# youthHan/HVRNet

Measured on AMD Instinct MI355X. Metric: VID frames/sec, R101 Faster-RCNN+HVR, 1000x600, 300 props, T=15, higher is better.
Workload: dtype bf16; 1 GPU; configs[2]: faster_rcnn_r101_hrnmp_c5 inference, clip mode; frames_per_window=15, proposals_per_frame=300, input=3x600x1000 padded to 608x1008, parallelism=dp1 independent clips, no collectives, windows_in_flight=12, clips_per_graph=3, key_frame_detections=300

## Files before the change

### hvrnet_amd/backbone.py

```python
import torch
import torch.nn as nn

from . import native
from .registry import BACKBONES, SHARED_HEADS

ARCH_SETTINGS = {50: (3, 4, 6, 3), 101: (3, 4, 23, 3), 152: (3, 8, 36, 3)}
STEM_KP = 192


def as_nhwc(x, dtype):
    v = x.permute(0, 2, 3, 1)
    if v.is_contiguous():
        return v if x.dtype == dtype else native.cast(v, dtype)
    return native.nchw_to_nhwc(x.contiguous(), dtype)


def as_logical(y):
    return y.permute(0, 3, 1, 2)


def fold_conv_bn(conv, bn, dtype):
    if bn is not None and conv.bias is None and dtype == torch.bfloat16 and conv.weight.is_cuda \
            and conv.weight.dtype == torch.float32 and conv.weight.is_contiguous() and not bn.training:
        from . import train_ops as TO
# ... 219 lines not shown
            if isinstance(m, nn.Conv2d):
                nn.init.kaiming_normal_(m.weight, mode='fan_out', nonlinearity='relu')
            elif isinstance(m, nn.BatchNorm2d):
                nn.init.constant_(m.weight, 1)
                nn.init.constant_(m.bias, 0)
        if self.zero_init_residual:
            for m in self.modules():
                if isinstance(m, Bottleneck):
                    nn.init.constant_(m.bn3.weight, 0)
        set_compute_dtype(self, self.compute_dtype)

    def _pack(self, dtype):
        w, b = fold_conv_bn(self.conv1, self.bn1, torch.float32)
        wp = torch.zeros((64, STEM_KP), dtype=torch.float32, device=w.device)
        wp[:, :147] = w.reshape(64, 147)
        wf = torch.zeros((64, 7, 8, 4), dtype=torch.float32, device=w.device)
        wf[:, :, :7, :3] = w
        if dtype == native.SPLIT:
            fused, fused_bias = native.stem_split_weights(wf.view(64, 7, 32)), native.stem_split_bias(b)
        else:
            fused, fused_bias = wf.view(64, 7, 32).to(dtype if dtype in (torch.bfloat16, torch.float16) else torch.bfloat16).contiguous(), b
        return dict(stem=(native.as_operand(wp, dtype), b), fused=fused, fused_bias=fused_bias)

    def out_shape_nhwc(self, B, H, W):
        if len(self.out_indices) != 1:
            return None
        last = self.out_indices[0]
        h, w = (H + 6 - 7) // 2 + 1, (W + 6 - 7) // 2 + 1
        h, w = (h + 2 - 3) // 2 + 1, (w + 2 - 3) // 2 + 1
        for i in range(last + 1):
            h, w = (h - 1) // self.strides[i] + 1, (w - 1) // self.strides[i] + 1
        return (B, h, w, 64 * 2 ** last * 4)

    def forward(self, x, out=None):
        if not x.is_cuda:
            raise NotImplementedError('ResNet runs on the GPU only (no CPU fallback)')
        p = self.packed(x.device)
        dt = self.compute_dtype
        if dt in (torch.bfloat16, torch.float16, native.SPLIT) and self.fused_stem:
            y = native.stem_fused(x.contiguous().float(), p['fused'], p['fused_bias'])
        else:
            cols, OH, OW = native.im2col_stem(x.contiguous().float(), dt, STEM_KP)
            if dt == native.SPLIT:
                y = native.gemm(cols, p['stem'][0], p['stem'][1], relu=True, out_f32=True).view(x.shape[0], OH, OW, 64)
                y = native.cast(native.maxpool3x3s2_nhwc(y), dt)
            else:
                y = native.gemm(cols, p['stem'][0], p['stem'][1], relu=True).view(x.shape[0], OH, OW, 64)
                y = native.maxpool3x3s2_nhwc(y)
        outs = []
        if out is not None:
            assert len(self.out_indices) == 1, 'out= needs a single returned map'
        for i, name in enumerate(self.res_layers):
            blocks = list(getattr(self, name))
            h1 = None
            for j, blk in enumerate(blocks):
                last = out is not None and i == self.out_indices[0] and j == len(blocks) - 1
                if j + 1 < len(blocks):
                    y, h1 = blk.forward_nhwc(y, h1=h1, nxt=blocks[j + 1])
                else:
                    y = blk.forward_nhwc(y, out=out if last else None, h1=h1)
            if i in self.out_indices:
                outs.append(as_logical(y))
            if out is not None and i == self.out_indices[0]:
                break
        return tuple(outs)

    def forward_train_nhwc(self, x):
        p = self.packed(x.device)
        dt = self.compute_dtype
        with torch.no_grad():
            if dt in (torch.bfloat16, torch.float16, native.SPLIT) and self.fused_stem:
                y = native.stem_fused(x.contiguous().float(), p['fused'], p['fused_bias'])
            else:
                cols, OH, OW = native.im2col_stem(x.contiguous().float(), dt, STEM_KP)
                y = native.gemm(cols, p['stem'][0], p['stem'][1], relu=True).view(x.shape[0], OH, OW, 64)
                y = native.maxpool3x3s2_nhwc(y)
            for i, name in enumerate(self.res_layers):
                if i + 1 <= self.frozen_stages:
                    for blk in getattr(self, name):
                        y = blk.forward_nhwc(y)
        for i, name in enumerate(self.res_layers):
            if i + 1 > self.frozen_stages:
                for blk in getattr(self, name):
                    y = blk.forward_train_nhwc(y)
        return y

    def train(self, mode=True):
# ... 67 lines not shown
```

### hvrnet_amd/csrc/capi.hip

```cpp
#include "../../include/hvr_hip.h"

#include <cmath>
#include <cstdarg>
#include <cstdio>
#include <cstdlib>
#include <cstring>
#include <string>

#include "common.h"
#include "gemm_params.h"
#include "relation_bt.h"

namespace hvr {
hipError_t run_transpose_pad(const void*, void*, int, int, long, long, int, hipStream_t);
hipError_t run_zero_fill(void*, size_t, hipStream_t);
hipError_t run_pack_conv_weights_multi(const void*, int, long, int, hipStream_t);
hipError_t run_transpose_multi(const void*, int, int, hipStream_t);
hipError_t run_im2col_t(const void*, void*, int, int, int, int, int, int, int, int, int, int, long, hipStream_t);
hipError_t run_relu_bwd_t(const void*, const void*, void*, void*, int, int, long, hipStream_t);
hipError_t run_splitk_reduce(const float*, float*, int, int, long, int, hipStream_t);
hipError_t run_unpack_conv_wgrads_multi(const void*, int, long, int, hipStream_t);
hipError_t run_splitk_reduce_bf16(const float*, void*, int, int, long, int, hipStream_t);
hipError_t run_splitk_reduce_f16(const float*, void*, int, int, long, int, hipStream_t);
hipError_t run_splitk_reduce_half_batched(const float*, void*, int, int, long, int, int, int, long, long, hipStream_t);
// ... 25 lines not shown
size_t tta_merge_proposals_workspace_bytes(int A, int T, int mx);
hipError_t run_tta_merge_proposals(const float*, const int*, int, int, int, const float*, const float*, const int*, float, int, float*, int*, void*,
                                   hipStream_t);
hipError_t run_tta_map_rois(const float*, int, int, int, const float*, const float*, const int*, float*, hipStream_t);
hipError_t run_tta_merge_dets(const float*, const float*, int, int, int, const float*, const float*, const int*, float*, float*, hipStream_t);
hipError_t run_mining_argreduce(const float*, int, int, long, const long long*, const long long*, long long*, hipStream_t);
hipError_t run_relation_dscore(const void*, const void*, const void*, const void*, void*, int, long, int, long, long, float, int, hipStream_t);
hipError_t run_im2col_stem(const float*, void*, int, int, int, int, int, int, int, hipStream_t);
hipError_t run_maxpool3x3s2(const void*, void*, int, int, int, int, int, int, int, hipStream_t);
hipError_t run_cast(const void*, void*, long, int, int, float, hipStream_t);
hipError_t run_permute(const void*, void*, int, int, int, int, int, int, hipStream_t);
hipError_t run_det_decode(const float*, int, int, int, int, const float*, int, const float*, const float*, float, float,
                          float, float, float*, float*, hipStream_t);
hipError_t run_roi_align_fwd(const void*, const float*, void*, int, int, int, int, int, int, int, float, int, int, int,
                             hipStream_t);
hipError_t run_roi_align_bwd(const float*, const float*, float*, int, int, int, int, int, int, float, int, int, hipStream_t);
size_t nms_workspace_bytes(int P, int n);
hipError_t run_nms_batched(const float*, int, int, float, int, int, int, long long*, int*, void*, hipStream_t, int band = 0,
                           int* band_done = nullptr);
hipError_t run_rpn_select(const void*, const void*, long, long, float*, const RpnParams&, int, hipStream_t);
hipError_t run_rpn_select_wide(const void*, const void*, long, long, float*, const RpnParams&, void*, hipStream_t);
size_t rpn_wide_workspace_bytes(int T, long n_anchor);
int rpn_wide_max_frames(int set);
int* rpn_wide_done_flags(void* wws, int T);
hipError_t run_rpn_gather(const float*, const long long*, const int*, int, int, int, int, int, float*, int*, hipStream_t);
hipError_t run_multiclass_nms(const float*, const float*, int, int, float, float, int, float*, long long*, int*, void*,
                              hipStream_t);
size_t multiclass_nms_workspace_bytes(int R, int ncls);
hipError_t run_soft_nms(const float*, int, float, int, float, float, float*, long long*, int*, hipStream_t);
hipError_t run_multiclass_soft_nms(const float*, const float*, int, int, int, float, float, int, float, float, int, float*, long long*, int*,
                                   void*, hipStream_t);
size_t multiclass_soft_nms_workspace_bytes(int P, int R, int ncls);
hipError_t run_stem_fused(const float*, const void*, const float*, void*, int, int, int, int, hipStream_t);
}

using namespace hvr;

static thread_local std::string g_err;

static int fail(int code, const char* fmt, ...) {
  char buf[512];
  va_list ap;
  va_start(ap, fmt);
  vsnprintf(buf, sizeof buf, fmt, ap);
  va_end(ap);
  g_err = buf;
  return code;
}
static int check_launch(hipError_t e, const char* what) {
  if (e == hipSuccess) return HVR_OK;
  if (e == hipErrorInvalidValue) return fail(HVR_EUNSUPPORTED, "%s: shape outside the implemented envelope", what);
  return fail(HVR_ELAUNCH, "%s: %s", what, hipGetErrorString(e));
}
static inline size_t align256(size_t b) { return (b + 255) & ~(size_t)255; }
static inline int elem_size(int dtype) { return (dtype == HVR_BF16 || dtype == HVR_F16) ? 2 : 4; }
static inline int kstep_elems(int dtype) { return (dtype == HVR_F32 || dtype == HVR_F16S) ? 32 : 64; }
static inline bool valid_dtype(int dtype) { return dtype >= HVR_F32 && dtype <= HVR_F16S; }
static inline bool aligned128(const void* p) { return (reinterpret_cast<uintptr_t>(p) & 127) == 0; }
static inline bool aligned16(const void* p) { return (reinterpret_cast<uintptr_t>(p) & 15) == 0; }

extern "C" {

int hvr_abi_version(void) { return 6; }
const char* hvr_last_error(void) { return g_err.c_str(); }

static int fill_linear(GemmParams& p, const void* A, const void* B, void* C, int M, int N, int K, long lda, long ldb,
// ... 366 lines not shown
    return fail(HVR_EUNSUPPORTED, "no fused tail + next conv kernel for C1=%d C2=%d Cout=%d Cn=%d", d->tail.C1, d->tail.C2, d->tail.Cout, d->Cn);
  return check_launch(run_expand(p, (hipStream_t)stream), "hvr_bottleneck_tail_next");
}

int hvr_conv2d_path(const hvr_conv_desc* d) {
  GemmParams p;
  int path = 0;
  const int rc = conv_params(d, p, path);
  if (rc) return rc;
  if (path == 0 && (d->tile_hint == 0 || d->tile_hint == kBigHint)) {
    p.tile_hint = 0;
    if (bigtile_supported(p, d->tile_hint == kBigHint)) return 3;
  }
  return path;
}

int hvr_im2col_stem(const float* img, void* cols, int B, int H, int W, int KP, int dtype, void* stream) {
  if (!img || !cols || B <= 0) return fail(HVR_EINVAL, "bad stem arguments");
  if (dtype == HVR_F16S && (KP % 32 || !aligned128(cols))) return fail(HVR_EINVAL, "split-half patch rows: KP %% 32 == 0, 128-byte aligned");
  if (KP < 147 || KP % kstep_elems(dtype)) return fail(HVR_EINVAL, "KP=%d must be >= 147 and a K-step multiple", KP);
  const int OH = (H + 6 - 7) / 2 + 1, OW = (W + 6 - 7) / 2 + 1;
  return check_launch(run_im2col_stem(img, cols, B, H, W, OH, OW, KP, dtype, (hipStream_t)stream), "hvr_im2col_stem");
}

int hvr_stem_fused_dtype(const float* img, const void* wpk, const float* bias, void* out, int B, int H, int W, int dtype, void* stream) {
  if (!img || !wpk || !bias || !out || B <= 0 || H < 7 || W < 7) return fail(HVR_EINVAL, "bad fused-stem arguments");
  if (dtype != HVR_BF16 && dtype != HVR_F16 && dtype != HVR_F16S) return fail(HVR_EUNSUPPORTED, "the fused stem computes on bf16, half or split-half operands");
  if (!aligned16(wpk) || !aligned16(out) || !aligned16(bias)) return fail(HVR_EINVAL, "fused stem operands must be 16-byte aligned");
  if (dtype == HVR_F16S && !aligned128(out)) return fail(HVR_EINVAL, "split-half stem output must be 128-byte aligned");
  return check_launch(run_stem_fused(img, wpk, bias, out, B, H, W, dtype, (hipStream_t)stream), "hvr_stem_fused");
}
int hvr_stem_fused(const float* img, const void* wpk, const float* bias, void* out, int B, int H, int W, void* stream) {
  return hvr_stem_fused_dtype(img, wpk, bias, out, B, H, W, HVR_BF16, stream);
}

int hvr_maxpool3x3s2_nhwc(const void* x, void* y, int B, int H, int W, int C, int dtype, void* stream) {
  if (!x || !y || C % 4) return fail(HVR_EINVAL, "bad maxpool arguments (C %% 4 == 0 required)");
  if (dtype == HVR_F16S) return fail(HVR_EUNSUPPORTED, "max pooling runs on f32 / bf16 / half maps");
  const int OH = (H + 2 - 3) / 2 + 1, OW = (W + 2 - 3) / 2 + 1;
  return check_launch(run_maxpool3x3s2(x, y, B, H, W, C, OH, OW, dtype, (hipStream_t)stream), "hvr_maxpool3x3s2_nhwc");
}

static int env_tile(const char* name) {
  const char* v = std::getenv(name);
  return v ? std::atoi(v) : 0;
}
static inline long rel_ldp(int Mk) { return ((long)Mk + 127) / 128 * 128; }

static int apply_slice_blocks() { return 4; }
static int apply_slices(int Mq, int Mk, int D) {
  const long tiles = (long)((Mq + 127) / 128) * ((D + 127) / 128);
  const int nblk = (int)(rel_ldp(Mk) / 128);
  if (tiles >= 96 || nblk < 8 || D % 8) return 1;
  const int per = apply_slice_blocks();
  return (nblk + per - 1) / per;
}

static int relation_apply_pass(const void* P, const void* Vt, float* mstat, float* lstat, float* partial, void* O, int64_t ldo,
                               int Mq, int Mk, int D, long ldp, int nt, int dtype, int staging, hipStream_t s) {
  const bool two_byte = dtype == HVR_BF16 || dtype == HVR_F16;
  constexpr int tile_apply = 0, gm_apply = 1;
#ifdef HVR_DEBUG_KNOBS
  static const int dbg_ld0 = env_tile("HVR_DBG_LD0");
#endif
  GemmParams p;
  int rc;
// ... 778 lines not shown
```

### hvrnet_amd/csrc/check_regs.py

```python
import re
import sys


def main(*paths):
    text = ''.join(open(p).read() for p in paths)
    blocks = re.split(r'remark: (?:\S+ )?Function Name: ', text)[1:]
    bad, seen = [], 0
    for b in blocks:
        name = b.split()[0]
        if name.startswith(('_ZN3hvr17expand_res_kernel', '_ZN3hvr19expand_split_kernel')):
            seen += 1
            spill = int(re.search(r'VGPRs Spill: (\d+)', b).group(1))
            scratch = int(re.search(r'ScratchSize \[bytes/lane\]: (\d+)', b).group(1))
            if spill or scratch:
                bad.append('%s: %d VGPRs spilled, %d bytes of scratch' % (name, spill, scratch))
            continue
        if name.startswith(('_ZN3hvr19mc_nms_', '_ZN3hvr15nms_', '_ZN3hvr16nms_', '_ZN3hvr17rpn_', '_ZN3hvr25relation_scores_bt', '_ZN3hvr14pc_tile_kernel', '_ZN3hvr15big_tile_kernel')) \
                or re.match(r'_ZN3hvr\d+(?:tta|soft_nms)_', name):
            seen += 1
            spill = int(re.search(r'VGPRs Spill: (\d+)', b).group(1))
            scratch = int(re.search(r'ScratchSize \[bytes/lane\]: (\d+)', b).group(1))
            allow = 32 if re.match(r'_ZN3hvr14pc_tile_kernelI(?:t|NS_5f16_tE)Li4ELi0E', name) else (256 if re.match(r'_ZN3hvr14pc_tile_kernelI(?:t|NS_5f16_tE)Li2ELi2E', name) else 0)
            if scratch > allow or (spill and not allow):
                bad.append('%s: %d VGPRs spilled, %d bytes of scratch' % (name, spill, scratch))
            continue
        m = re.match(r'_ZN3hvr11tile_kernelI(?:t|f|NS_5f16_tE|NS_6f16s_tE)Li(\d+)ELi(\d+)ELi(\d+)ELi(\d+)ELi(\d+)ELb([01])ELb([01])ELi(\d+)E', name)
        if not m:
            continue
        wm, wn, fm, fn, epi, glds, respre, ns = [int(x) for x in m.groups()]
        spill = int(re.search(r'VGPRs Spill: (\d+)', b).group(1))
        bn = wn * fn * 16
        split_pipe = 'f16s_t' in name and ns > 2 and not (wm == 3 and fn == 8)
        untracked = epi == 2 or (ns > 2 and respre == 1 and bn != 256) or split_pipe
        if untracked:
            seen += 1
            if spill:
                bad.append('%s: %d VGPRs spilled' % (name, spill))
    if not seen:
        sys.exit('check_regs: no kernel recognised in the remarks (format change?)')
    if bad:
        sys.exit('check_regs: these kernels must not spill:\n  ' + '\n  '.join(bad))
    print('check_regs: %d kernels checked (untracked loads / serial sweeps / big accumulator tiles), none spills' % seen)

# ... 4 lines not shown
```

### hvrnet_amd/csrc/stem.hip

```cpp
#include "common.h"

namespace hvr {

#ifndef HVR_ST_PH
#define HVR_ST_PH 3
#endif
#ifndef HVR_ST_PW
#define HVR_ST_PW 16
#endif
constexpr int ST_PH = HVR_ST_PH, ST_PW = HVR_ST_PW;
constexpr int ST_CH = 2 * ST_PH + 1, ST_CW = 2 * ST_PW + 1;
constexpr int ST_NCONV = ST_CH * ST_CW;
constexpr int ST_FRAGS = (ST_NCONV + 15) / 16;
constexpr int ST_IR = 2 * (ST_CH - 1) + 7, ST_IC = 2 * (ST_CW - 1) + 7;
constexpr int ST_PCOLS = 72;
constexpr int ST_CROW = 68;
constexpr int ST_PATCH_BYTES = (ST_IR + 3) * ST_PCOLS * 4 * 2;
constexpr int ST_CONV_BYTES = ST_FRAGS * 16 * ST_CROW * 2;

template <typename T>
__global__ __launch_bounds__(256) void stem_fused_kernel(const float* __restrict__ img, const uint4* __restrict__ wpk,
                                                         const float* __restrict__ bias, T* __restrict__ out, int H,
                                                         int W, int CH, int CW, int PH, int PW) {
  extern __shared__ __attribute__((aligned(16))) char smem[];
  T* patch = reinterpret_cast<T*>(smem);
  T* cbuf = reinterpret_cast<T*>(smem + ST_PATCH_BYTES);
  const int tid = threadIdx.x, lane = tid & 63, wave = tid >> 6;
  const int px0 = blockIdx.x * ST_PW, py0 = blockIdx.y * ST_PH, b = blockIdx.z;
  const int cy0 = 2 * py0 - 1, cx0 = 2 * px0 - 1;
  const int iy0 = 2 * cy0 - 3, ix0 = 2 * cx0 - 3;

  uint4 wf[4][7];
#pragma unroll
// ... 169 lines not shown

  for (int i = tid; i < ST_PH * ST_PW * 4; i += 256) {
    const int ch = i & 3, q = i >> 2, qy = q / ST_PW, qx = q - qy * ST_PW;
    const int py = py0 + qy, px = px0 + qx;
    if (py >= PH || px >= PW) continue;
    float best[8];
#pragma unroll
    for (int e = 0; e < 8; ++e) best[e] = -INFINITY;
#pragma unroll
    for (int dy = 0; dy < 3; ++dy) {
      const int gy = 2 * py - 1 + dy;
      if ((unsigned)gy >= (unsigned)CH) continue;
#pragma unroll
      for (int dx = 0; dx < 3; ++dx) {
        const int gx = 2 * px - 1 + dx;
        if ((unsigned)gx >= (unsigned)CW) continue;
        const float* src = cbuf + ((gy - cy0) * ST_CW + (gx - cx0)) * ST_CROWF + ch * 8;
        const float4 a = *reinterpret_cast<const float4*>(src), c = *reinterpret_cast<const float4*>(src + 4);
        best[0] = fmaxf(best[0], a.x); best[1] = fmaxf(best[1], a.y); best[2] = fmaxf(best[2], a.z); best[3] = fmaxf(best[3], a.w);
        best[4] = fmaxf(best[4], c.x); best[5] = fmaxf(best[5], c.y); best[6] = fmaxf(best[6], c.z); best[7] = fmaxf(best[7], c.w);
      }
    }
    uint4 h, l;
    split2(best[0], best[1], h.x, l.x); split2(best[2], best[3], h.y, l.y);
    split2(best[4], best[5], h.z, l.z); split2(best[6], best[7], h.w, l.w);
    char* dst = out + (((long)b * PH + py) * PW + px) * 256 + half * 128 + ch * 16;
    *reinterpret_cast<uint4*>(dst) = h;
    *reinterpret_cast<uint4*>(dst + kSplitPlane) = l;
  }
  __syncthreads();
  }
}

hipError_t run_stem_fused(const float* img, const void* wpk, const float* bias, void* out, int B, int H, int W, int dtype, hipStream_t s) {
  const int CH = (H + 6 - 7) / 2 + 1, CW = (W + 6 - 7) / 2 + 1;
  const int PH = (CH + 2 - 3) / 2 + 1, PW = (CW + 2 - 3) / 2 + 1;
  constexpr int lds = ST_PATCH_BYTES + ST_CONV_BYTES;
  static std::atomic<unsigned> attr_dev{0};
  per_device_once(attr_dev, [&] {
    (void)hipFuncSetAttribute(reinterpret_cast<const void*>(stem_fused_kernel<bf16_t>), hipFuncAttributeMaxDynamicSharedMemorySize, lds);
    (void)hipFuncSetAttribute(reinterpret_cast<const void*>(stem_fused_kernel<f16_t>), hipFuncAttributeMaxDynamicSharedMemorySize, lds);
  });
  dim3 grid((PW + ST_PW - 1) / ST_PW, (PH + ST_PH - 1) / ST_PH, B);
  if (dtype == DT_F16S) {
    static std::atomic<unsigned> sattr_dev{0};
    per_device_once(sattr_dev, [&] {
      (void)hipFuncSetAttribute(reinterpret_cast<const void*>(stem_fused_split_kernel), hipFuncAttributeMaxDynamicSharedMemorySize, ST_SPLIT_LDS);
    });
    hipLaunchKernelGGL(stem_fused_split_kernel, grid, dim3(256), ST_SPLIT_LDS, s, img, (const uint4*)wpk, bias, (char*)out, H, W, CH, CW, PH, PW);
    return hipGetLastError();
  }
  if (dtype == DT_F16)
    hipLaunchKernelGGL(stem_fused_kernel<f16_t>, grid, dim3(256), lds, s, img, (const uint4*)wpk, bias, (f16_t*)out, H, W, CH, CW, PH, PW);
  else
    hipLaunchKernelGGL(stem_fused_kernel<bf16_t>, grid, dim3(256), lds, s, img, (const uint4*)wpk, bias, (bf16_t*)out, H, W, CH, CW, PH, PW);
  return hipGetLastError();
}

}
```

### hvrnet_amd/native.py

```python
import contextlib
import ctypes
import math
import os
import subprocess

import torch

_HERE = os.path.dirname(os.path.abspath(__file__))
LIB_PATH = os.path.join(_HERE, 'libhvr_hip.so')
HEADER_PATH = os.path.join(os.path.dirname(_HERE), 'include', 'hvr_hip.h')

HVR_F32, HVR_BF16, HVR_F16, HVR_F16S = 0, 1, 2, 3
ABI_VERSION = 6
SPLIT = torch.int32
COMPUTE_DTYPES = (torch.bfloat16, torch.float16, SPLIT, torch.float32)
DTYPE_NAMES = {torch.bfloat16: 'bf16', torch.float16: 'f16', SPLIT: 'f16x2', torch.float32: 'f32'}
LAYOUT_NCHW, LAYOUT_NHWC = 0, 1

STAGING = 1
TILE_HINT = 0


class HvrError(RuntimeError):
    pass
# ... 37 lines not shown
class RpnDesc(ctypes.Structure):
    _fields_ = [('cls', ctypes.c_void_p), ('reg', ctypes.c_void_p),
                ('T', ctypes.c_int32), ('H', ctypes.c_int32), ('W', ctypes.c_int32),
                ('A', ctypes.c_int32), ('anchor_stride', ctypes.c_int32),
                ('base_anchors', ctypes.c_void_p), ('means', ctypes.c_void_p), ('stds', ctypes.c_void_p),
                ('img_h', ctypes.c_float), ('img_w', ctypes.c_float), ('wh_ratio_clip', ctypes.c_float),
                ('nms_pre', ctypes.c_int32), ('nms_post', ctypes.c_int32), ('max_num', ctypes.c_int32),
                ('nms_thr', ctypes.c_float),
                ('proposals', ctypes.c_void_p), ('counts', ctypes.c_void_p),
                ('cls_pitch', ctypes.c_int32), ('reg_pitch', ctypes.c_int32)]


_vp, _i, _f, _i64, _sz = ctypes.c_void_p, ctypes.c_int, ctypes.c_float, ctypes.c_int64, ctypes.c_size_t
SYMBOLS = {
    'hvr_abi_version': (_i, []),
    'hvr_last_error': (ctypes.c_char_p, []),
    'hvr_gemm': (_i, [ctypes.POINTER(GemmDesc), _vp]),
    'hvr_gemm_fewrow_workspace_bytes': (_sz, [ctypes.POINTER(GemmDesc)]),
    'hvr_gemm_splitk_workspace_bytes': (_sz, [_i, _i, _i, _i]),
    'hvr_gemm_splitk': (_i, [ctypes.POINTER(GemmDesc), _vp, _sz, _vp]),
    'hvr_gemm_splitk_batched_workspace_bytes': (_sz, [_i, _i, _i, _i, _i]),
    'hvr_gemm_splitk_batched': (_i, [ctypes.POINTER(GemmDesc), _i, _i64, _i64, _i64, _vp, _sz, _vp]),
    'hvr_conv2d_nhwc': (_i, [ctypes.POINTER(ConvDesc), _vp]),
    'hvr_conv2d_path': (_i, [ctypes.POINTER(ConvDesc)]),
    'hvr_conv2d_splitk_workspace_bytes': (_sz, [ctypes.POINTER(ConvDesc)]),
    'hvr_bottleneck_tail': (_i, [ctypes.POINTER(TailDesc), _vp]),
    'hvr_bottleneck_tail_supported': (_i, [ctypes.POINTER(TailDesc)]),
    'hvr_bottleneck_tail_next': (_i, [ctypes.POINTER(TailNextDesc), _vp]),
    'hvr_bottleneck_tail_next_supported': (_i, [ctypes.POINTER(TailNextDesc)]),
    'hvr_im2col_stem': (_i, [_vp, _vp, _i, _i, _i, _i, _i, _vp]),
    'hvr_maxpool3x3s2_nhwc': (_i, [_vp, _vp, _i, _i, _i, _i, _i, _vp]),
    'hvr_stem_fused': (_i, [_vp, _vp, _vp, _vp, _i, _i, _i, _vp]),
    'hvr_stem_fused_dtype': (_i, [_vp, _vp, _vp, _vp, _i, _i, _i, _i, _vp]),
    'hvr_relation_workspace_bytes': (_sz, [_i, _i, _i, _i]),
    'hvr_relation_fwd': (_i, [_vp, _i64, _vp, _i64, _vp, _i64, _vp, _i64, _i, _i, _i, _f, _i, _i, _vp, _sz, _vp]),
    'hvr_relation_grouped_workspace_bytes': (_sz, [_i, _i, _i, _i, _i]),
    'hvr_relation_fwd_grouped': (_i, [_vp, _i64, _i64, _vp, _i64, _i64, _vp, _i64, _i64, _vp, _i64, _i64, _i, _i, _i, _i, _f, _i, _i, _i, _vp, _sz, _vp]),
    'hvr_relation_probs_workspace_bytes': (_sz, [_i, _i]),
    'hvr_relation_probs': (_i, [_vp, _i64, _vp, _i64, _vp, _i64, _i, _i, _i, _f, _i, _i, _vp, _sz, _vp]),
    'hvr_relation_dscore': (_i, [_vp, _vp, _vp, _i64, _vp, _i64, _vp, _i, _i64, _i, _f, _i, _vp]),
    'hvr_relu_bwd': (_i, [_vp, _vp, _vp, _i64, _i, _vp]),
    'hvr_im2col_nhwc': (_i, [_vp, _vp, _i, _i, _i, _i, _i, _i, _i, _i, _i, _vp]),
    'hvr_im2col_t': (_i, [_vp, _vp, _i64, _i, _i, _i, _i, _i, _i, _i, _i, _i, _vp]),
    'hvr_relu_bwd_t': (_i, [_vp, _vp, _vp, _vp, _i64, _i, _i, _i, _vp]),
    'hvr_scale_rows': (_i, [_vp, _vp, _vp, _i, _i64, _i, _vp]),
    'hvr_sgd_workspace_bytes': (_sz, []),
    'hvr_sgd_step': (_i, [_vp, _vp, _vp, _i64, _f, _f, _f, _f, _f, _vp, _sz, _i, _vp]),
    'hvr_colsum_workspace_bytes': (_sz, [_i, _i]),
    'hvr_colsum': (_i, [_vp, _vp, _i, _i, _i64, _i, _vp, _sz, _vp]),
    'hvr_pack_conv_weight': (_i, [_vp, _vp, _vp, _i, _i, _i, _i, _i, _vp]),
    'hvr_pack_conv_weights_multi': (_i, [_vp, _i, _i64, _i, _vp]),
    'hvr_transpose_multi': (_i, [_vp, _i, _i, _vp]),
    'hvr_unpack_conv_wgrad': (_i, [_vp, _vp, _vp, _i, _i, _i, _i, _i, _vp]),
    'hvr_unpack_conv_wgrads_multi': (_i, [_vp, _i, _i64, _i, _vp]),
    'hvr_det_loss': (_i, [_vp, _i, _i, _i, _i, _vp, _vp, _vp, _vp, _i, _f, _f, _f, _vp, _vp, _vp]),
    'hvr_det_loss_sampled': (_i, [_vp, _i, _i, _i, _i, _vp, _vp, _vp, _vp, _i, _vp, _f, _vp, _vp, _vp]),
    'hvr_max_iou_assign_workspace_bytes': (_sz, [_i, _i]),
    'hvr_max_iou_assign': (_i, [_vp, _i, _i, _vp, _i, _vp, _f, _f, _f, _f, _vp, _vp, _vp, _sz, _vp]),
    'hvr_sample_pos_neg': (_i, [_vp, _vp, _i, _i, _i, _f, _vp, _vp, _vp]),
    'hvr_box_targets': (_i, [_vp, _i, _i, _vp, _vp, _vp, _vp, _vp, _i, _vp, _vp, _f, _i, _vp, _vp, _vp, _vp, _vp]),
    'hvr_rpn_loss': (_i, [_vp, _i, _i, _i, _vp, _vp, _vp, _vp, _vp, _f, _vp, _vp, _vp]),
    'hvr_ce_rows': (_i, [_vp, _i, _i, _i, _vp, _i, _vp, _vp]),
    'hvr_triplet_margin': (_i, [_vp, _i64, _vp, _i64, _i, _i, _i, _vp, _vp, _vp, _i, _f, _i, _vp, _sz, _vp, _vp, _vp, _vp]),
    'hvr_ingest_frame': (_i, [_vp, _i, _i, _i64, _vp, _i, _i, _i, _i, _vp, _vp, _i, _vp]),
    'hvr_ingest_frame_flip': (_i, [_vp, _i, _i, _i64, _vp, _i, _i, _i, _i, _vp, _vp, _i, _i, _vp]),
    'hvr_merge_aug_proposals_workspace_bytes': (_sz, [_i, _i, _i]),
# ... 367 lines not shown
    fake = 1 << 20
    d = ConvDesc(x=fake, w=fake, y=fake, B=B, H=H, W=W, Cin=Cin, Cout=Cout, KH=k, KW=k, stride=stride, pad=pad, dil=dil,
                 bias=fake if bias else None, resid=fake if resid else None, relu=1, out_f32=int(out_f32),
                 dtype={torch.bfloat16: HVR_BF16, torch.float16: HVR_F16, SPLIT: HVR_F16S}.get(dtype, HVR_F32), staging=STAGING,
                 tile_hint=tile, zero=fake)
    return int(lib().hvr_conv2d_path(ctypes.byref(d)))


def im2col_stem(img, dtype, kp=192):
    _need_cuda(img)
    assert img.dtype == torch.float32 and img.is_contiguous()
    B, _, H, W = img.shape
    OH, OW = (H + 6 - 7) // 2 + 1, (W + 6 - 7) // 2 + 1
    cols = torch.empty((B * OH * OW, kp), dtype=torch.float32 if dtype == SPLIT else dtype, device=img.device)
    _check(lib().hvr_im2col_stem(_ptr(img), _ptr(cols), B, H, W, kp, _dt(cols), _stream()), 'hvr_im2col_stem')
    return (cast(cols, SPLIT) if dtype == SPLIT else cols), OH, OW


def stem_fused(img, wpk, bias):
    _need_cuda(img, wpk, bias)
    assert img.dtype == torch.float32 and img.is_contiguous() and wpk.dtype in (torch.bfloat16, torch.float16)
    split = wpk.dim() == 4
    assert tuple(wpk.shape) == ((2, 64, 7, 32) if split else (64, 7, 32)) and (not split or wpk.dtype == torch.float16) and wpk.is_contiguous()
    B, _, H, W = img.shape
    CH, CW = (H + 6 - 7) // 2 + 1, (W + 6 - 7) // 2 + 1
    PH, PW = (CH + 2 - 3) // 2 + 1, (CW + 2 - 3) // 2 + 1
    out = torch.empty((B, PH, PW, 64), dtype=SPLIT if split else wpk.dtype, device=img.device)
    with _span('stem', 2.0 * B * CH * CW * 64 * 147):
        _check(lib().hvr_stem_fused_dtype(_ptr(img), _ptr(wpk), _ptr(bias), _ptr(out), B, H, W, HVR_F16S if split else _dt(wpk), _stream()),
               'hvr_stem_fused')
    return out


def stem_split_weights(wf):
    wf = wf * (SPLIT_WEIGHT_SCALE * SPLIT_ACT_SCALE)
    hi = wf.half()
    lo = (wf - hi.float()).half()
    return torch.stack([hi, lo], 0).contiguous()


def stem_split_bias(b):
    return (b * SPLIT_ACT_SCALE).contiguous()


def maxpool3x3s2_nhwc(x):
    _need_cuda(x)
    if x.dtype == SPLIT:
        return cast(maxpool3x3s2_nhwc(cast(x, torch.float32)), SPLIT)
    B, H, W, C = x.shape
    OH, OW = (H + 2 - 3) // 2 + 1, (W + 2 - 3) // 2 + 1
    y = torch.empty((B, OH, OW, C), dtype=x.dtype, device=x.device)
    _check(lib().hvr_maxpool3x3s2_nhwc(_ptr(x), _ptr(y), B, H, W, C, _dt(x), _stream()), 'hvr_maxpool3x3s2_nhwc')
    return y


_ws_cache = {}


_fewrow = [False]


@contextlib.contextmanager
def fewrow_split(on=True):
    prev = _fewrow[0]
    _fewrow[0] = bool(on)
    try:
# ... 696 lines not shown
```

### include/hvr_hip.h

```cpp
#ifndef HVR_HIP_H_
#define HVR_HIP_H_

#include <stddef.h>
#include <stdint.h>

#ifdef __cplusplus
extern "C" {
#endif

#define HVR_OK 0
#define HVR_EINVAL (-1)
#define HVR_EUNSUPPORTED (-2)
#define HVR_ELAUNCH (-3)
#define HVR_EWORKSPACE (-4)

#define HVR_F32 0
#define HVR_BF16 1
#define HVR_F16 2
#define HVR_F16S 3

#define HVR_LAYOUT_NCHW 0
#define HVR_LAYOUT_NHWC 1

int hvr_abi_version(void);
// ... 29 lines not shown
  const float* bias;
  const void* resid;
  int32_t relu, out_f32, dtype, staging, tile_hint;
  const void* zero;
  void* ws; size_t ws_bytes;
  float alpha, beta;
} hvr_conv_desc;
int hvr_conv2d_nhwc(const hvr_conv_desc* d, void* stream);
size_t hvr_conv2d_splitk_workspace_bytes(const hvr_conv_desc* d);
int hvr_conv2d_path(const hvr_conv_desc* d);

typedef struct hvr_tail_desc {
  const void* h; const void* x; const void* w; void* y;
  int32_t B, OH, OW, C1, H2, W2, C2, stride2, Cout;
  const float* bias;
  int32_t relu, dtype;
} hvr_tail_desc;
int hvr_bottleneck_tail(const hvr_tail_desc* d, void* stream);
int hvr_bottleneck_tail_supported(const hvr_tail_desc* d);

typedef struct hvr_tail_next_desc {
  hvr_tail_desc tail;
  const void* resid;
  const void* wn; const float* bias_n; void* hn;
  int32_t Cn;
  float alpha, beta;
} hvr_tail_next_desc;
int hvr_bottleneck_tail_next(const hvr_tail_next_desc* d, void* stream);
int hvr_bottleneck_tail_next_supported(const hvr_tail_next_desc* d);

int hvr_im2col_stem(const float* img, void* cols, int B, int H, int W, int KP, int dtype, void* stream);
int hvr_stem_fused(const float* img, const void* wpk, const float* bias, void* out, int B, int H, int W, void* stream);
int hvr_stem_fused_dtype(const float* img, const void* wpk, const float* bias, void* out, int B, int H, int W, int dtype, void* stream);
int hvr_maxpool3x3s2_nhwc(const void* x, void* y, int B, int H, int W, int C, int dtype, void* stream);

size_t hvr_relation_workspace_bytes(int Mq, int Mk, int D, int dtype);
int hvr_relation_fwd(const void* Q, int64_t ldq, const void* K, int64_t ldk, const void* V, int64_t ldv,
                     void* O, int64_t ldo, int Mq, int Mk, int D, float scale, int dtype, int staging,
                     void* ws, size_t ws_bytes, void* stream);

size_t hvr_relation_grouped_workspace_bytes(int groups, int Mq, int Mk, int D, int dtype);
int hvr_relation_fwd_grouped(const void* Q, int64_t ldq, int64_t gsq, const void* K, int64_t ldk, int64_t gsk,
                             const void* V, int64_t ldv, int64_t gsv, void* O, int64_t ldo, int64_t gso, int groups,
                             int Mq, int Mk, int D, float scale, int dtype, int staging, int exact, void* ws, size_t ws_bytes, void* stream);

size_t hvr_relation_probs_workspace_bytes(int Mq, int Mk);
int hvr_relation_probs(const void* Q, int64_t ldq, const void* K, int64_t ldk, void* P, int64_t ldp, int Mq, int Mk, int D,
                       float scale, int dtype, int staging, void* ws, size_t ws_bytes, void* stream);
int hvr_relation_dscore(const void* P, const void* dP, const void* dO, int64_t ldgo, const void* O, int64_t ldo, void* dS,
                        int Mq, int64_t ldp, int D, float scale, int dtype, void* stream);

int hvr_relu_bwd(const void* dY, const void* Y, void* dZ, int64_t n, int dtype, void* stream);
size_t hvr_colsum_workspace_bytes(int M, int N);
int hvr_colsum(const void* dY, float* db, int M, int N, int64_t ld, int dtype, void* ws, size_t ws_bytes, void* stream);
int hvr_det_loss(const float* logits, int ldl, int cls_off, int reg_off, int ncls, const int64_t* labels, const float* label_weights,
                 const float* bbox_targets, const float* bbox_weights, int R, float beta, float w_cls, float w_bbox, float* out3,
                 float* dlogits, void* stream);

int hvr_im2col_nhwc(const void* x, void* cols, int B, int H, int W, int Cin, int KH, int KW, int pad, int dil, int dtype, void* stream);
int hvr_im2col_t(const void* x, void* colsT, int64_t ldt, int B, int H, int W, int Cin, int KH, int KW, int pad, int dil, int dtype, void* stream);
int hvr_relu_bwd_t(const void* dY, const void* Y, void* dZ, void* dZt, int64_t ldt, int R, int C, int dtype, void* stream);
int hvr_scale_rows(const void* w, const float* scale, void* out, int R, int64_t C, int dtype, void* stream);
int hvr_pack_conv_weight(const float* w, const float* scale, void* out, int Cout, int Cin, int KH, int KW, int out_dtype, void* stream);
int hvr_unpack_conv_wgrad(const float* dw, const float* scale, float* out, int Cout, int Cin, int KH, int KW, int accumulate, void* stream);
typedef struct { const float* w; const float* scale; void* out; int64_t first; int32_t Cout, Cin, KK, pad_; } hvr_pack_item;
typedef struct { const void* src; void* dst; int64_t lds, ldd; int32_t R, C, first_tile, tiles_c, dcols, pad_; } hvr_transpose_item;
// ... 96 lines not shown
```

Before: 184.8 frames/s.

## Add persistent fused stem kernel with ring-buffered patches and optional conv1 fusion

Adds a persistent stem kernel in which each workgroup walks a contiguous range of tiles. It keeps input rows in an LDS ring, prefetches the next tile's rows while the MFMAs run on the current one, and reuses the overlapping patch rows instead of reloading them. The default bf16/half stem path now routes to this kernel. An optional variant also runs the first bottleneck conv1 (1x1) on the pooled tile in LDS, but it is gated off by default. The change adds complexity in the LDS layout and register pressure, and lowers occupancy.

```diff
diff --git a/hvrnet_amd/backbone.py b/hvrnet_amd/backbone.py
--- a/hvrnet_amd/backbone.py
+++ b/hvrnet_amd/backbone.py
@@ -275,12 +275,19 @@
             h, w = (h - 1) // self.strides[i] + 1, (w - 1) // self.strides[i] + 1
         return (B, h, w, 64 * 2 ** last * 4)
 
+    fuse_stem_next = False
+
     def forward(self, x, out=None):
         if not x.is_cuda:
             raise NotImplementedError('ResNet runs on the GPU only (no CPU fallback)')
         p = self.packed(x.device)
         dt = self.compute_dtype
-        if dt in (torch.bfloat16, torch.float16, native.SPLIT) and self.fused_stem:
+        h1_first = None
+        first = getattr(self, self.res_layers[0])[0]
+        if dt in (torch.bfloat16, torch.float16) and self.fused_stem and self.fuse_stem_next and first.conv1_stride == 1:
+            c1 = first.packed(x.device)['c1']
+            y, h1_first = native.stem_fused_next(x.contiguous().float(), p['fused'], p['fused_bias'], c1[0], c1[1])
+        elif dt in (torch.bfloat16, torch.float16, native.SPLIT) and self.fused_stem:
             y = native.stem_fused(x.contiguous().float(), p['fused'], p['fused_bias'])
         else:
             cols, OH, OW = native.im2col_stem(x.contiguous().float(), dt, STEM_KP)
@@ -295,7 +302,7 @@
             assert len(self.out_indices) == 1, 'out= needs a single returned map'
         for i, name in enumerate(self.res_layers):
             blocks = list(getattr(self, name))
-            h1 = None
+            h1 = h1_first if i == 0 else None
             for j, blk in enumerate(blocks):
                 last = out is not None and i == self.out_indices[0] and j == len(blocks) - 1
                 if j + 1 < len(blocks):
diff --git a/hvrnet_amd/csrc/capi.hip b/hvrnet_amd/csrc/capi.hip
--- a/hvrnet_amd/csrc/capi.hip
+++ b/hvrnet_amd/csrc/capi.hip
@@ -81,6 +81,7 @@
                                    void*, hipStream_t);
 size_t multiclass_soft_nms_workspace_bytes(int P, int R, int ncls);
 hipError_t run_stem_fused(const float*, const void*, const float*, void*, int, int, int, int, hipStream_t);
+hipError_t run_stem_fused_next(const float*, const void*, const float*, const void*, const float*, void*, void*, int, int, int, int, int, hipStream_t);
 }
 
 using namespace hvr;
@@ -513,6 +514,21 @@
 }
 int hvr_stem_fused(const float* img, const void* wpk, const float* bias, void* out, int B, int H, int W, void* stream) {
   return hvr_stem_fused_dtype(img, wpk, bias, out, B, H, W, HVR_BF16, stream);
+}
+int hvr_stem_fused_next(const float* img, const void* wpk, const float* bias, const void* w1, const float* bias1, void* out, void* out_h1, int B, int H,
+                        int W, int dtype, int variant, void* stream) {
+  if (!img || !wpk || !bias || !out || B <= 0 || H < 7 || W < 7) return fail(HVR_EINVAL, "bad fused-stem arguments");
+  if (dtype != HVR_BF16 && dtype != HVR_F16 && dtype != HVR_F16S) return fail(HVR_EUNSUPPORTED, "the fused stem computes on bf16, half or split-half operands");
+  if (variant != HVR_STEM_AUTO && variant != HVR_STEM_PERSISTENT && variant != HVR_STEM_ONE_TILE) return fail(HVR_EINVAL, "bad fused-stem variant %d", variant);
+  if (!aligned16(wpk) || !aligned16(out) || !aligned16(bias)) return fail(HVR_EINVAL, "fused stem operands must be 16-byte aligned");
+  if (dtype == HVR_F16S && !aligned128(out)) return fail(HVR_EINVAL, "split-half stem output must be 128-byte aligned");
+  if (dtype == HVR_F16S && variant == HVR_STEM_PERSISTENT) return fail(HVR_EUNSUPPORTED, "the split-half stem has the one-tile kernel only");
+  if (w1) {
+    if (dtype == HVR_F16S || variant == HVR_STEM_ONE_TILE) return fail(HVR_EUNSUPPORTED, "conv1 rides on the persistent bf16 / half stem only");
+    if (!bias1 || !out_h1 || !aligned16(w1) || !aligned16(bias1) || !aligned16(out_h1)) return fail(HVR_EINVAL, "fused stem + conv1: w1, bias1, out_h1 must be given and 16-byte aligned");
+  }
+  return check_launch(run_stem_fused_next(img, wpk, bias, w1, w1 ? bias1 : nullptr, out, w1 ? out_h1 : nullptr, B, H, W, dtype, variant, (hipStream_t)stream),
+                      "hvr_stem_fused_next");
 }
 
 int hvr_maxpool3x3s2_nhwc(const void* x, void* y, int B, int H, int W, int C, int dtype, void* stream) {
diff --git a/hvrnet_amd/csrc/check_regs.py b/hvrnet_amd/csrc/check_regs.py
--- a/hvrnet_amd/csrc/check_regs.py
+++ b/hvrnet_amd/csrc/check_regs.py
@@ -9,6 +9,13 @@
     for b in blocks:
         name = b.split()[0]
         if name.startswith(('_ZN3hvr17expand_res_kernel', '_ZN3hvr19expand_split_kernel')):
+            seen += 1
+            spill = int(re.search(r'VGPRs Spill: (\d+)', b).group(1))
+            scratch = int(re.search(r'ScratchSize \[bytes/lane\]: (\d+)', b).group(1))
+            if spill or scratch:
+                bad.append('%s: %d VGPRs spilled, %d bytes of scratch' % (name, spill, scratch))
+            continue
+        if name.startswith('_ZN3hvr28stem_fused_kernel_persistent'):
             seen += 1
             spill = int(re.search(r'VGPRs Spill: (\d+)', b).group(1))
             scratch = int(re.search(r'ScratchSize \[bytes/lane\]: (\d+)', b).group(1))
diff --git a/hvrnet_amd/csrc/stem.hip b/hvrnet_amd/csrc/stem.hip
--- a/hvrnet_amd/csrc/stem.hip
+++ b/hvrnet_amd/csrc/stem.hip
@@ -1,4 +1,5 @@
 #include "common.h"
+#include <cstdio>
 
 namespace hvr {
 
@@ -234,7 +235,259 @@
   }
 }
 
-hipError_t run_stem_fused(const float* img, const void* wpk, const float* bias, void* out, int B, int H, int W, int dtype, hipStream_t s) {
+constexpr int SP_SLOTS = 24, SP_PITCH = 78, SP_ROWB = SP_PITCH * 8;
+constexpr int SP_MIRROR = 7;
+constexpr int SP_QUADS = 19, SP_ROWS = 12;
+constexpr int SP_PATCH_BYTES = (SP_SLOTS + SP_MIRROR + 1) * SP_ROWB;
+constexpr int SP_CSLOTS = 7;
+constexpr int SP_CONV_BYTES = SP_CSLOTS * ST_CW * ST_CROW * 2;
+constexpr int SP_PROW = 72;
+constexpr int SP_POOL_BYTES = ST_PH * ST_PW * SP_PROW * 2;
+constexpr int SP_BIAS_BYTES = 2 * 64 * 4;
+constexpr int sp_lds_bytes(bool next) { return SP_PATCH_BYTES + SP_CONV_BYTES + SP_BIAS_BYTES + (next ? 2 * SP_POOL_BYTES : 0); }
+constexpr int sp_wg_per_cu(bool next) { return next ? 2 : 3; }
+static_assert(ST_PH == 3 && ST_PW == 16, "the persistent stem's rings are laid out for 3 x 16 pooled tiles");
+static_assert(SP_QUADS * SP_ROWS <= 256 && 3 * sp_lds_bytes(false) <= 160 * 1024 && 2 * sp_lds_bytes(true) <= 160 * 1024, "persistent stem: load items / LDS budget");
+
+__device__ __forceinline__ void sp_lds_barrier() {
+  asm volatile("s_waitcnt lgkmcnt(0)" ::: "memory");
+  __builtin_amdgcn_s_barrier();
+  asm volatile("" ::: "memory");
+}
+
+template <bool WIDE>
+__device__ __forceinline__ void sp_load(const float* __restrict__ ib, int H, int W, int u0, int xa, int r, float (&v)[3][4]) {
+  const int iy = u0 + r + 2;
+  const int yc = iy < 0 ? 0 : (iy >= H ? H - 1 : iy);
+  const long plane = (long)H * W;
+  if constexpr (WIDE) {
+    const int xc = xa < 0 ? 0 : (xa > W - 4 ? W - 4 : xa);
+    const float* src = ib + (long)yc * W + xc;
+#pragma unroll
+    for (int c = 0; c < 3; ++c) {
+      const float4 t = *reinterpret_cast<const float4*>(src + c * plane);
+      v[c][0] = t.x; v[c][1] = t.y; v[c][2] = t.z; v[c][3] = t.w;
+    }
+  } else {
+#pragma unroll
+    for (int e = 0; e < 4; ++e) {
+      const int x = xa + e;
+      const int xc = x < 0 ? 0 : (x >= W ? W - 1 : x);
+      const float* src = ib + (long)yc * W + xc;
+#pragma unroll
+      for (int c = 0; c < 3; ++c) v[c][e] = src[c * plane];
+    }
+  }
+}
+
+template <typename T>
+__device__ __forceinline__ void sp_store(char* patch, int H, int W, int u0, int xa, int r, int q, bool item, const float (&v)[3][4]) {
+  const int iy = u0 + r + 2;
+  const bool rowok = (unsigned)iy < (unsigned)H;
+  uint32_t w[8];
+#pragma unroll
+  for (int e = 0; e < 4; ++e) {
+    const bool ok = rowok && (unsigned)(xa + e) < (unsigned)W && 4 * q - 3 + e <= 2 * (ST_CW - 1) + 6;
+    w[2 * e] = pack2<T>(ok ? v[0][e] : 0.f, ok ? v[1][e] : 0.f);
+    w[2 * e + 1] = pack2<T>(ok ? v[2][e] : 0.f, 0.f);
+  }
+  const int slot = item ? (u0 + r + 2 * SP_SLOTS) % SP_SLOTS : SP_SLOTS + SP_MIRROR;
+  char* dst = patch + slot * SP_ROWB + (4 * q + 1) * 8;
+  *reinterpret_cast<uint2*>(dst) = make_uint2(w[0], w[1]);
+  *reinterpret_cast<uint4*>(dst + 8) = make_uint4(w[2], w[3], w[4], w[5]);
+  *reinterpret_cast<uint2*>(dst + 24) = make_uint2(w[6], w[7]);
+  if (slot < SP_MIRROR) {
+    dst += SP_SLOTS * SP_ROWB;
+    *reinterpret_cast<uint2*>(dst) = make_uint2(w[0], w[1]);
+    *reinterpret_cast<uint4*>(dst + 8) = make_uint4(w[2], w[3], w[4], w[5]);
+    *reinterpret_cast<uint2*>(dst + 24) = make_uint2(w[6], w[7]);
+  }
+}
+
+typedef unsigned short sp_u16x2 __attribute__((ext_vector_type(2)));
+__device__ __forceinline__ uint32_t sp_pkmax(uint32_t a, uint32_t b) {
+  return __builtin_bit_cast(uint32_t, __builtin_elementwise_max(__builtin_bit_cast(sp_u16x2, a), __builtin_bit_cast(sp_u16x2, b)));
+}
+
+template <typename T, bool WIDE, bool NEXT>
+__global__ __launch_bounds__(256, sp_wg_per_cu(NEXT)) void stem_fused_kernel_persistent(
+    const float* __restrict__ img, const uint4* __restrict__ wpk, const float* __restrict__ bias, const uint4* __restrict__ w1,
+    const float* __restrict__ bias1, T* __restrict__ out, T* __restrict__ out_h1, int H, int W, int CH, int CW, int PH, int PW,
+    int nstrips, int ntile_y, int ntiles) {
+  extern __shared__ __attribute__((aligned(16))) char smem[];
+  char* patch = smem;
+  T* cbuf = reinterpret_cast<T*>(smem + SP_PATCH_BYTES);
+  float* sbias = reinterpret_cast<float*>(smem + SP_PATCH_BYTES + SP_CONV_BYTES);
+  T* pbuf = reinterpret_cast<T*>(smem + SP_PATCH_BYTES + SP_CONV_BYTES + SP_BIAS_BYTES);
+  T* hbuf = reinterpret_cast<T*>(smem + SP_PATCH_BYTES + SP_CONV_BYTES + SP_BIAS_BYTES + SP_POOL_BYTES);
+  const int tid = threadIdx.x, lane = tid & 63, wave = tid >> 6;
+  const int fi = lane & 15, fg = lane >> 4;
+  const int nwg = gridDim.x;
+  const int t0 = (int)((long)blockIdx.x * ntiles / nwg), t1 = (int)((long)(blockIdx.x + 1) * ntiles / nwg);
+  if (t0 >= t1) return;
+
+  const int fh = wave & 1, nh = wave >> 1;
+  uint4 wf[2][7];
+#pragma unroll
+  for (int j = 0; j < 2; ++j)
+#pragma unroll
+    for (int ky = 0; ky < 7; ++ky) wf[j][ky] = wpk[(((nh * 2 + j) * 16 + fi) * 7 + ky) * 4 + fg];
+  uint4 w1f[2];
+  if constexpr (NEXT) {
+#pragma unroll
+    for (int kk = 0; kk < 2; ++kk) w1f[kk] = w1[(wave * 16 + fi) * 8 + kk * 4 + fg];
+  }
+  if (tid < 64) sbias[tid] = bias[tid];
+  else if (NEXT && tid < 128) sbias[tid] = bias1[tid - 64];
+
+  const int lr = tid / SP_QUADS < SP_ROWS ? tid / SP_QUADS : SP_ROWS - 1, lq = tid % SP_QUADS;
+  const bool litem = tid < SP_QUADS * SP_ROWS;
+
+  int ty = t0 % ntile_y, strip = (t0 / ntile_y) % nstrips, b = t0 / (ntile_y * nstrips);
+  {
+    const float* ib = img + (long)b * 3 * H * W;
+    const int xa = 4 * ST_PW * strip - 8 + 4 * lq;
+    float va[3][4], vb[3][4];
+    sp_load<WIDE>(ib, H, W, 12 * ty - 12, xa, lr, va);
+    sp_load<WIDE>(ib, H, W, 12 * ty, xa, lr, vb);
+    sp_store<T>(patch, H, W, 12 * ty - 12, xa, lr, lq, litem, va);
+    sp_store<T>(patch, H, W, 12 * ty, xa, lr, lq, litem, vb);
+  }
+  __builtin_amdgcn_s_waitcnt(0x0F70);
+  sp_lds_barrier();
+
+  float4 bv[2];
+#pragma unroll
+  for (int j = 0; j < 2; ++j) bv[j] = *reinterpret_cast<const float4*>(sbias + (nh * 2 + j) * 16 + fg * 4);
+  float4 bv1 = make_float4(0.f, 0.f, 0.f, 0.f);
+  if constexpr (NEXT) bv1 = *reinterpret_cast<const float4*>(sbias + 64 + wave * 16 + fg * 4);
+
+  bool restart = true;
+  int pty = 0, pstrip = 0, pb = 0;
+  auto flush_h1 = [&](int fb, int fstrip, int fty) {
+    for (int i = tid; i < ST_PH * ST_PW * 8; i += 256) {
+      const int ch = i & 7, q = i >> 3, py = ST_PH * fty + (q >> 4), px = ST_PW * fstrip + (q & 15);
+      const uint4 v = *reinterpret_cast<const uint4*>(hbuf + q * SP_PROW + ch * 8);
+#ifndef HVR_SP_DBG_NOSTORE
+      if (py < PH && px < PW) *reinterpret_cast<uint4*>(out_h1 + (((long)fb * PH + py) * PW + px) * 64 + ch * 8) = v;
+#else
+      if (v.x == 0x12345u) out_h1[0] = (T)1;
+#endif
+    }
+  };
+  for (int t = t0; t < t1; ++t) {
+    const bool has_next = t + 1 < t1;
+    int nty = ty + 1, nstrip = strip, nb = b;
+    if (nty == ntile_y) {
+      nty = 0;
+      if (++nstrip == nstrips) { nstrip = 0; ++nb; }
+    }
+    const float* nib = img + (long)(has_next ? nb : b) * 3 * H * W;
+    const int nxa = 4 * ST_PW * (has_next ? nstrip : strip) - 8 + 4 * lq;
+    const int nu0 = 12 * (has_next ? nty : ty);
+    float pv[3][4];
+#ifndef HVR_SP_DBG_NOLOAD
+    sp_load<WIDE>(nib, H, W, nu0, nxa, lr, pv);
+#endif
+
+    const int cbeg = 6 * ty - (restart ? 1 : 0), cx0 = 2 * ST_PW * strip - 1;
+    const int npix = (restart ? 7 : 6) * ST_CW, nfr = (npix + 15) >> 4;
+#ifndef HVR_SP_DBG_NOMFMA
+    for (int f = (fh + t) & 1; f < nfr; f += 2) {
+      const int p = f * 16 + fi;
+      const int pc = p < npix ? p : npix - 1;
+      const int cyl = pc / ST_CW, cxl = pc - cyl * ST_CW;
+      const int cy = cbeg + cyl;
+      const char* abase = patch + ((2 * cy - 5 + 2 * SP_SLOTS) % SP_SLOTS) * SP_ROWB + (2 * cxl + 4 + 2 * fg) * 8;
+      f32x4 acc[2];
+#pragma unroll
+      for (int j = 0; j < 2; ++j) acc[j] = f32x4{0.f, 0.f, 0.f, 0.f};
+#pragma unroll
+      for (int ky = 0; ky < 7; ++ky) {
+        const uint4 a = *reinterpret_cast<const uint4*>(abase + ky * SP_ROWB);
+#pragma unroll
+        for (int j = 0; j < 2; ++j) acc[j] = mfma_half<T>(wf[j][ky], a, acc[j]);
+      }
+      if (p < npix) {
+        T* crow = cbuf + (((cy + 1) % SP_CSLOTS) * ST_CW + cxl) * ST_CROW;
+        const bool inmap = (unsigned)cy < (unsigned)CH && (unsigned)(cx0 + cxl) < (unsigned)CW;
+#pragma unroll
+        for (int j = 0; j < 2; ++j) {
+          const int n = (nh * 2 + j) * 16 + fg * 4;
+          const uint32_t lo = pack2<T>(fmaxf(acc[j][0] + bv[j].x, 0.f), fmaxf(acc[j][1] + bv[j].y, 0.f));
+          const uint32_t hi = pack2<T>(fmaxf(acc[j][2] + bv[j].z, 0.f), fmaxf(acc[j][3] + bv[j].w, 0.f));
+          *reinterpret_cast<uint2*>(crow + n) = make_uint2(inmap ? lo : 0u, inmap ? hi : 0u);
+        }
+      }
+    }
+#endif
+    sp_lds_barrier();
+
+#ifndef HVR_SP_DBG_NOLOAD
+    {
+      sp_store<T>(patch, H, W, nu0, nxa, lr, lq, litem && has_next, pv);
+      if (has_next && nty == 0) {
+        sp_load<WIDE>(nib, H, W, -12, nxa, lr, pv);
+        sp_store<T>(patch, H, W, -12, nxa, lr, lq, litem, pv);
+      }
+    }
+#endif
+
+    const int py0 = ST_PH * ty, px0 = ST_PW * strip;
+#ifndef HVR_SP_DBG_NOPOOL
+    const int rs0 = (6 * ty) % SP_CSLOTS;
+    for (int i = tid; i < ST_PH * ST_PW * 8; i += 256) {
+      const int ch = i & 7, q = i >> 3, qy = q >> 4, qx = q & 15;
+      uint4 best = make_uint4(0u, 0u, 0u, 0u);
+#pragma unroll
+      for (int dy = 0; dy < 3; ++dy) {
+        int rs = rs0 + 2 * qy + dy;
+        rs = rs >= 2 * SP_CSLOTS ? rs - 2 * SP_CSLOTS : (rs >= SP_CSLOTS ? rs - SP_CSLOTS : rs);
+        const T* src = cbuf + (rs * ST_CW + 2 * qx) * ST_CROW + ch * 8;
+#pragma unroll
+        for (int dx = 0; dx < 3; ++dx) {
+          const uint2 a = *reinterpret_cast<const uint2*>(src + dx * ST_CROW), c = *reinterpret_cast<const uint2*>(src + dx * ST_CROW + 4);
+          best.x = sp_pkmax(best.x, a.x); best.y = sp_pkmax(best.y, a.y); best.z = sp_pkmax(best.z, c.x); best.w = sp_pkmax(best.w, c.y);
+        }
+      }
+      const int py = py0 + qy, px = px0 + qx;
+#ifndef HVR_SP_DBG_NOSTORE
+      if (py < PH && px < PW) *reinterpret_cast<uint4*>(out + (((long)b * PH + py) * PW + px) * 64 + ch * 8) = best;
+#endif
+      if constexpr (NEXT) *reinterpret_cast<uint4*>(pbuf + q * SP_PROW + ch * 8) = best;
+    }
+    if constexpr (NEXT) {
+      if (t > t0) flush_h1(pb, pstrip, pty);
+    }
+#endif
+
+    sp_lds_barrier();
+
+    if constexpr (NEXT) {
+      const int n = wave * 16 + fg * 4;
+#ifndef HVR_SP_DBG_NOC1
+#pragma unroll
+      for (int pf = 0; pf < ST_PH; ++pf) {
+        const T* prow = pbuf + (pf * 16 + fi) * SP_PROW + fg * 8;
+        const uint4 x0 = *reinterpret_cast<const uint4*>(prow), x1 = *reinterpret_cast<const uint4*>(prow + 32);
+        f32x4 acc = mfma_half<T>(w1f[0], x0, f32x4{0.f, 0.f, 0.f, 0.f});
+        acc = mfma_half<T>(w1f[1], x1, acc);
+        const float v[4] = {fmaxf(acc[0] + bv1.x, 0.f), fmaxf(acc[1] + bv1.y, 0.f), fmaxf(acc[2] + bv1.z, 0.f), fmaxf(acc[3] + bv1.w, 0.f)};
+        store4(hbuf + (pf * 16 + fi) * SP_PROW + n, v);
+      }
+#endif
+    }
+    pty = ty; pstrip = strip; pb = b;
+    restart = nty == 0;
+    ty = nty; strip = nstrip; b = nb;
+  }
+  if constexpr (NEXT) {
+    sp_lds_barrier();
+    flush_h1(pb, pstrip, pty);
+  }
+}
+
+static hipError_t run_stem_one_tile(const float* img, const void* wpk, const float* bias, void* out, int B, int H, int W, int dtype, hipStream_t s) {
   const int CH = (H + 6 - 7) / 2 + 1, CW = (W + 6 - 7) / 2 + 1;
   const int PH = (CH + 2 - 3) / 2 + 1, PW = (CW + 2 - 3) / 2 + 1;
   constexpr int lds = ST_PATCH_BYTES + ST_CONV_BYTES;
@@ -259,4 +512,62 @@
   return hipGetLastError();
 }
 
-}
+static int device_cus() {
+  static std::atomic<int> cus[kMaxDevices];
+  int d = -1;
+  (void)hipGetDevice(&d);
+  const bool slot = d >= 0 && d < kMaxDevices;
+  int n = slot ? cus[d].load(std::memory_order_acquire) : 0;
+  if (n > 0) return n;
+  hipDeviceProp_t prop;
+  if (hipGetDeviceProperties(&prop, d < 0 ? 0 : d) != hipSuccess || prop.multiProcessorCount <= 0) return 0;
+  n = prop.multiProcessorCount;
+  if (slot) cus[d].store(n, std::memory_order_release);
+  return n;
+}
+
+template <typename T, bool WIDE, bool NEXT>
+static hipError_t launch_stem_persistent(const float* img, const void* wpk, const float* bias, const void* w1, const float* bias1, void* out,
+                                         void* out_h1, int B, int H, int W, hipStream_t s) {
+  const int CH = (H + 6 - 7) / 2 + 1, CW = (W + 6 - 7) / 2 + 1;
+  const int PH = (CH + 2 - 3) / 2 + 1, PW = (CW + 2 - 3) / 2 + 1;
+  const int nstrips = (PW + ST_PW - 1) / ST_PW, ntile_y = (PH + ST_PH - 1) / ST_PH;
+  const long ntiles = (long)B * nstrips * ntile_y;
+  const int cus = device_cus();
+  if (cus <= 0 || ntiles > 0x7fffffffL) return hipErrorInvalidValue;
+  const auto kern = stem_fused_kernel_persistent<T, WIDE, NEXT>;
+  static std::atomic<unsigned> attr_dev{0};
+  per_device_once(attr_dev, [&] { (void)hipFuncSetAttribute(reinterpret_cast<const void*>(kern), hipFuncAttributeMaxDynamicSharedMemorySize, sp_lds_bytes(NEXT)); });
+  int per_cu = 0;
+  if (hipOccupancyMaxActiveBlocksPerMultiprocessor(&per_cu, reinterpret_cast<const void*>(kern), 256, sp_lds_bytes(NEXT)) != hipSuccess || per_cu <= 0) per_cu = 1;
+#ifdef HVR_SP_DBG_PERCU
+  static std::atomic<int> told{0};
+  if (!told.exchange(1)) fprintf(stderr, "stem persistent: %d CUs, %d workgroups per CU by the occupancy query\n", cus, per_cu);
+  per_cu = HVR_SP_DBG_PERCU;
+#endif
+  const long slots = (long)cus * per_cu;
+  const int grid = (int)(ntiles < slots ? ntiles : slots);
+  hipLaunchKernelGGL(kern, dim3(grid), dim3(256), sp_lds_bytes(NEXT), s, img, (const uint4*)wpk, bias, (const uint4*)w1, bias1, (T*)out, (T*)out_h1, H, W, CH,
+                     CW, PH, PW, nstrips, ntile_y, (int)ntiles);
+  return hipGetLastError();
+}
+
+hipError_t run_stem_fused_next(const float* img, const void* wpk, const float* bias, const void* w1, const float* bias1, void* out, void* out_h1,
+                               int B, int H, int W, int dtype, int variant, hipStream_t s) {
+  if (dtype == DT_F16S || variant == 2) {
+    if (w1) return hipErrorInvalidValue;
+    return run_stem_one_tile(img, wpk, bias, out, B, H, W, dtype, s);
+  }
+  const bool wide = (W & 3) == 0 && (reinterpret_cast<uintptr_t>(img) & 15) == 0;
+#define HVR_SP_LAUNCH(T, WIDE, NEXT) launch_stem_persistent<T, WIDE, NEXT>(img, wpk, bias, w1, bias1, out, out_h1, B, H, W, s)
+#define HVR_SP_PICK(T) (wide ? (w1 ? HVR_SP_LAUNCH(T, true, true) : HVR_SP_LAUNCH(T, true, false)) : (w1 ? HVR_SP_LAUNCH(T, false, true) : HVR_SP_LAUNCH(T, false, false)))
+  return dtype == DT_F16 ? HVR_SP_PICK(f16_t) : HVR_SP_PICK(bf16_t);
+#undef HVR_SP_PICK
+#undef HVR_SP_LAUNCH
+}
+
+hipError_t run_stem_fused(const float* img, const void* wpk, const float* bias, void* out, int B, int H, int W, int dtype, hipStream_t s) {
+  return run_stem_fused_next(img, wpk, bias, nullptr, nullptr, out, nullptr, B, H, W, dtype, 0, s);
+}
+
+}
diff --git a/hvrnet_amd/native.py b/hvrnet_amd/native.py
--- a/hvrnet_amd/native.py
+++ b/hvrnet_amd/native.py
@@ -93,6 +93,7 @@
     'hvr_maxpool3x3s2_nhwc': (_i, [_vp, _vp, _i, _i, _i, _i, _i, _vp]),
     'hvr_stem_fused': (_i, [_vp, _vp, _vp, _vp, _i, _i, _i, _vp]),
     'hvr_stem_fused_dtype': (_i, [_vp, _vp, _vp, _vp, _i, _i, _i, _i, _vp]),
+    'hvr_stem_fused_next': (_i, [_vp, _vp, _vp, _vp, _vp, _vp, _vp, _i, _i, _i, _i, _i, _vp]),
     'hvr_relation_workspace_bytes': (_sz, [_i, _i, _i, _i]),
     'hvr_relation_fwd': (_i, [_vp, _i64, _vp, _i64, _vp, _i64, _vp, _i64, _i, _i, _i, _f, _i, _i, _vp, _sz, _vp]),
     'hvr_relation_grouped_workspace_bytes': (_sz, [_i, _i, _i, _i, _i]),
@@ -526,6 +527,33 @@
     return out
 
 
+STEM_AUTO, STEM_PERSISTENT, STEM_ONE_TILE = 0, 1, 2
+
+
+def stem_fused_next(img, wpk, bias, w1=None, bias1=None, variant=STEM_AUTO):
+    _need_cuda(img, wpk, bias)
+    assert img.dtype == torch.float32 and img.is_contiguous() and wpk.dtype in (torch.bfloat16, torch.float16)
+    split = wpk.dim() == 4
+    assert tuple(wpk.shape) == ((2, 64, 7, 32) if split else (64, 7, 32)) and (not split or wpk.dtype == torch.float16) and wpk.is_contiguous()
+    B, _, H, W = img.shape
+    CH, CW = (H + 6 - 7) // 2 + 1, (W + 6 - 7) // 2 + 1
+    PH, PW = (CH + 2 - 3) // 2 + 1, (CW + 2 - 3) // 2 + 1
+    out = torch.empty((B, PH, PW, 64), dtype=SPLIT if split else wpk.dtype, device=img.device)
+    h1 = None
+    work = 2.0 * B * CH * CW * 64 * 147
+    if w1 is not None:
+        _need_cuda(w1, bias1)
+        assert not split and w1.dtype == wpk.dtype and w1.numel() == 64 * 64 and w1.shape[0] == 64 and w1.is_contiguous()
+        assert bias1.dtype == torch.float32 and bias1.numel() == 64 and bias1.is_contiguous()
+        h1 = torch.empty((B, PH, PW, 64), dtype=wpk.dtype, device=img.device)
+        work += 2.0 * B * PH * PW * 64 * 64
+    with _span('stem', work):
+        _check(lib().hvr_stem_fused_next(_ptr(img), _ptr(wpk), _ptr(bias), _ptr(w1) if w1 is not None else None,
+                                         _ptr(bias1) if w1 is not None else None, _ptr(out), _ptr(h1) if h1 is not None else None,
+                                         B, H, W, HVR_F16S if split else _dt(wpk), int(variant), _stream()), 'hvr_stem_fused_next')
+    return out, h1
+
+
 def stem_split_weights(wf):
     wf = wf * (SPLIT_WEIGHT_SCALE * SPLIT_ACT_SCALE)
     hi = wf.half()
diff --git a/include/hvr_hip.h b/include/hvr_hip.h
--- a/include/hvr_hip.h
+++ b/include/hvr_hip.h
@@ -85,6 +85,9 @@
 int hvr_im2col_stem(const float* img, void* cols, int B, int H, int W, int KP, int dtype, void* stream);
 int hvr_stem_fused(const float* img, const void* wpk, const float* bias, void* out, int B, int H, int W, void* stream);
 int hvr_stem_fused_dtype(const float* img, const void* wpk, const float* bias, void* out, int B, int H, int W, int dtype, void* stream);
+enum { HVR_STEM_AUTO = 0, HVR_STEM_PERSISTENT = 1, HVR_STEM_ONE_TILE = 2 };
+int hvr_stem_fused_next(const float* img, const void* wpk, const float* bias, const void* w1, const float* bias1, void* out, void* out_h1,
+                        int B, int H, int W, int dtype, int variant, void* stream);
 int hvr_maxpool3x3s2_nhwc(const void* x, void* y, int B, int H, int W, int C, int dtype, void* stream);
 
 size_t hvr_relation_workspace_bytes(int Mq, int Mk, int D, int dtype);
```

Result: no change. 186.4 frames/s (median of 6 runs) (+0.9%).
